# hukaixuan19970627/yolov5_obb

Hardware: AMD Instinct MI355X
Metric: val.py img/s (hot path: non_max_suppression_obb, bs16) + NMS ms/img @100k cand, DOTAv1.5 1024^2, 1/2/4/8 GPU (higher is better)
Workload: dtype f16; 1 GPU; DOTAv1.5 1024^2 bs16 (BASELINE metric; configs[1] thresholds): yolov5 OBB head output (16,64512,201) fp16, 4 distinct tensors rotated (cold: 1.66 GB working set) -> non_max_suppression_obb (conf .25, iou .45, multi_label, max_det 1500), val.py --task speed hot path = dt[2] of val.py; global_batch=16, anchors_per_image=64512, nc=16, detections_per_batch=3734, parallelism=dp1 (images sharded, no data-path collective)

## Files before the change

### include/obb_hip.h

```cpp
#ifndef OBB_HIP_H
#define OBB_HIP_H

#include <stddef.h>
#include <stdint.h>

#ifdef __cplusplus
extern "C" {
#endif

#define OBB_OK 0
#define OBB_ERR_BAD_ARG (-1)
#define OBB_ERR_WORKSPACE (-2)
#define OBB_ERR_LAUNCH (-3)
#define OBB_ERR_INTERNAL (-4)
#define OBB_ERR_NO_DEVICE (-5)

#define OBB_NMS_DROP_SMALL 1

const char* obb_version(void);
int obb_device_info(int* cu_count, int* wave_size, char* arch_name, int arch_name_len);
int obb_nms_set_max_grid(int max_workgroups);

#define OBB_PROF_STAGES 8
int obb_profile_enable(int on);
// ... 37 lines not shown
#define OBB_NMS_SORT_LDS_HINT 6144
#define OBB_NMS_SORT_LDS_MAX 8192
size_t obb_nms_obb_workspace_bytes(int64_t bs, int64_t cap_img, int64_t nc, int agnostic);
int obb_non_max_suppression_obb(const void* pred, int dtype, int64_t bs, int64_t A, int64_t no, float conf_thres,
                                float iou_thres, const int32_t* classes_host, int n_classes, int agnostic, int multi_label,
                                int64_t max_det, int64_t max_nms, float max_wh, const float* extra8, int64_t n_extra,
                                int64_t cap_img, int64_t expected_cand, float* out, int out_packed, int64_t* out_count,
                                int64_t* status, void* ws, size_t ws_bytes, void* stream);
int obb_non_max_suppression_obb_col(const void* pred, const void* objcol, int dtype, int64_t bs, int64_t A, int64_t no,
                                    float conf_thres, float iou_thres, const int32_t* classes_host, int n_classes, int agnostic,
                                    int multi_label, int64_t max_det, int64_t max_nms, float max_wh, const float* extra8,
                                    int64_t n_extra, int64_t cap_img, int64_t expected_cand, float* out, int out_packed,
                                    int64_t* out_count, int64_t* status, void* ws, size_t ws_bytes, void* stream);

size_t obb_nms_obb_state_bytes(int64_t bs);
int obb_non_max_suppression_obb_st(const void* pred, const void* objcol, int dtype, int64_t bs, int64_t A, int64_t no,
                                   float conf_thres, float iou_thres, const int32_t* classes_host, int n_classes, int agnostic,
                                   int multi_label, int64_t max_det, int64_t max_nms, float max_wh, const float* extra8,
                                   int64_t n_extra, int64_t cap_img, int64_t expected_cand, float* out, int out_packed,
                                   int64_t* out_count, int64_t* status, void* ws, size_t ws_bytes, void* state, size_t state_bytes,
                                   void* stream);

int obb_non_max_suppression_obb_head(int nl, const void* const* conv_out, int dtype, int64_t bs, int64_t na, int64_t no,
                                     const int64_t* ny, const int64_t* nx, const float* anchors_px_host, const float* strides_host,
                                     float conf_thres, float iou_thres, const int32_t* classes_host, int n_classes, int agnostic,
                                     int multi_label, int64_t max_det, int64_t max_nms, float max_wh, const float* extra8,
                                     int64_t n_extra, int64_t cap_img, int64_t expected_cand, float* out, int out_packed,
                                     int64_t* out_count, int64_t* status, void* ws, size_t ws_bytes, void* state, size_t state_bytes,
                                     void* stream);

// ... 84 lines not shown
```

### yolov5_obb_amd/_lib.py

```python
import ctypes as C
import os
import threading

import torch

_HERE = os.path.dirname(os.path.abspath(__file__))
LIB_PATH = os.environ.get("OBB_HIP_LIB") or os.path.join(_HERE, "libobb_hip.so")

OBB_OK = 0
OBB_NMS_DROP_SMALL = 1
_ERR = {-1: "bad argument", -2: "workspace missing or too small", -3: "kernel launch failed",
        -4: "internal error", -5: "no usable HIP device"}

_lib = None
_lock = threading.RLock()

_vp, _i64, _i32, _f32, _sz = C.c_void_p, C.c_int64, C.c_int, C.c_float, C.c_size_t

SIGNATURES = {
    "obb_version": (C.c_char_p, []),
    "obb_device_info": (_i32, [C.POINTER(_i32), C.POINTER(_i32), C.c_char_p, _i32]),
    "obb_nms_set_max_grid": (_i32, [_i32]),
    "obb_profile_enable": (_i32, [_i32]),
    "obb_profile_collect": (_i32, [_vp, _vp, _i32]),
# ... 3 lines not shown
    "obb_nms_poly_f32": (_i32, [_vp, _i64, _i64, _f32, _i64, _vp, _vp, _vp, _sz, _vp]),
    "obb_merge_nms_poly_f64": (_i32, [_vp, _i64, _vp, _vp, _i64, C.c_double, _vp, _vp, _vp, _sz, _vp]),
    "obb_merge_nms_poly_all_f64": (_i32, [_vp, _i64, _vp, _vp, _i64, C.c_double, _vp, _vp, _vp, _sz, _vp]),
    "obb_merge_nms_hbb_f64": (_i32, [_vp, _i64, _i64, _vp, _vp, _i64, C.c_double, _vp, _vp, _vp, _sz, _vp]),
    "obb_task1_parse_tiles": (_i64, [_vp, _i64, _i64, _vp, _vp, _vp, _vp, _vp, _vp]),
    "obb_task1_format_rows": (_i64, [_vp, _vp, _vp, _vp, _vp, _i64, _vp, _i64]),
    "obb_task1_parse_dets": (_i64, [_vp, _i64, _i64, _vp, _vp, _vp, _vp]),
    "obb_task1_parse_gt": (_i64, [_vp, _i64, _i64, _vp, _vp, _vp, _vp]),
    "obb_eval_best_gt_f64": (_i32, [_vp, _vp, _i64, _vp, _vp, _i64, _vp, _vp, _vp]),
    "obb_nms_obb_workspace_bytes": (_sz, [_i64, _i64, _i64, _i32]),
    "obb_non_max_suppression_obb": (_i32, [_vp, _i32, _i64, _i64, _i64, _f32, _f32, _vp, _i32, _i32, _i32, _i64, _i64, _f32,
                                           _vp, _i64, _i64, _i64, _vp, _i32, _vp, _vp, _vp, _sz, _vp]),
    "obb_non_max_suppression_obb_col": (_i32, [_vp, _vp, _i32, _i64, _i64, _i64, _f32, _f32, _vp, _i32, _i32, _i32, _i64, _i64, _f32,
                                               _vp, _i64, _i64, _i64, _vp, _i32, _vp, _vp, _vp, _sz, _vp]),
    "obb_nms_obb_state_bytes": (_sz, [_i64]),
    "obb_non_max_suppression_obb_st": (_i32, [_vp, _vp, _i32, _i64, _i64, _i64, _f32, _f32, _vp, _i32, _i32, _i32, _i64, _i64, _f32,
                                              _vp, _i64, _i64, _i64, _vp, _i32, _vp, _vp, _vp, _sz, _vp, _sz, _vp]),
    "obb_non_max_suppression_obb_head": (_i32, [_i32, _vp, _i32, _i64, _i64, _i64, _vp, _vp, _vp, _vp, _f32, _f32, _vp, _i32, _i32, _i32,
                                                _i64, _i64, _f32, _vp, _i64, _i64, _i64, _vp, _i32, _vp, _vp, _vp, _sz, _vp, _sz, _vp]),
    "obb_loss_workspace_bytes": (_sz, [_vp, _i64]),
    "obb_loss_build_targets": (_i32, [_vp, _vp, _i64, _i64, _vp, _vp, _sz, _vp]),
    "obb_loss_export_targets": (_i32, [_vp, _i64, _i32, _i64, _vp, _vp, _vp, _vp, _vp, _vp, _sz, _vp]),
    "obb_loss_forward": (_i32, [_vp, _vp, _i32, _vp, _i64, _i64, _vp, _vp, _sz, _vp]),
    "obb_loss_backward": (_i32, [_vp, _vp, _i32, _vp, _i64, _i64, _vp, _vp, _vp, _sz, _vp]),
    "obb_detect_decode": (_i32, [_vp, _i32, _i64, _i64, _i64, _i64, _i64, _vp, _f32, _vp, _vp, _i64, _i64, _vp]),
    "obb_detect_decode_col": (_i32, [_vp, _i32, _i64, _i64, _i64, _i64, _i64, _vp, _f32, _vp, _vp, _i64, _i64, _vp, _vp]),
    "obb_detect_decode_levels": (_i32, [_i32, _vp, _i32, _i64, _i64, _i64, _vp, _vp, _vp, _vp, _vp, _vp, _i64, _vp, _vp]),
    "obb_csl_encode_f32": (_i32, [_vp, _i64, _i32, C.c_double, C.c_double, _vp, _vp]),
    "obb_rbox2poly_f32": (_i32, [_vp, _i64, _i64, _vp, _vp, _vp]),
    "obb_val_postprocess_f32": (_i32, [_vp, _i64, _f32, _f32, _f32, _vp, _vp, _vp, _vp, _vp]),
# ... 202 lines not shown
```

### yolov5_obb_amd/csrc/nms.hip

```cpp
#include <hip/hip_runtime.h>
#include <cstring>
#include <stdint.h>
#include <stdlib.h>
#include <stdio.h>
#include <string.h>
#include <hip/hip_fp16.h>
#include "launch_once.h"
#include "obb_device.h"
#include "nms_core.h"
#include "nms_mk.h"
#include "obb_hip.h"
#include "psrs_sort.h"
#include "nms_small.h"
#include "segsort.h"

namespace obb {

enum { PROF_DECODE = 0, PROF_SEGSORT, PROF_PREP, PROF_STEPS, PROF_GATHER, PROF_NMS_SORT, PROF_NMS_PREP, PROF_NMS_STEPS, PROF_N };
struct ProfState {
  int on = 0;
  static constexpr int kMax = 8192;
  hipEvent_t ev0[kMax], ev1[kMax];
  int id[kMax];
  int created = 0, used = 0;
// ... 965 lines not shown
                                         out_packed, out_count, status, ws, ws_bytes, stream);
}

int obb_non_max_suppression_obb_col(const void* pred, const void* objcol, int dtype, int64_t bs, int64_t A, int64_t no,
                                    float conf_thres, float iou_thres, const int32_t* classes_host, int n_classes, int agnostic,
                                    int multi_label, int64_t max_det, int64_t max_nms, float max_wh, const float* extra8,
                                    int64_t n_extra, int64_t cap_img, int64_t expected_cand, float* out, int out_packed,
                                    int64_t* out_count, int64_t* status, void* ws, size_t ws_bytes, void* stream) {
  return run_nms_obb(pred, objcol, dtype, bs, A, no, conf_thres, iou_thres, classes_host, n_classes, agnostic, multi_label, max_det,
                     max_nms, max_wh, extra8, n_extra, cap_img, expected_cand, out, out_packed ? 1 : 0, out_count, status, ws, ws_bytes,
                     (hipStream_t)stream);
}

size_t obb_nms_obb_state_bytes(int64_t bs) { return bs < 1 ? 0 : obb_state_bytes(bs); }

int obb_non_max_suppression_obb_st(const void* pred, const void* objcol, int dtype, int64_t bs, int64_t A, int64_t no,
                                   float conf_thres, float iou_thres, const int32_t* classes_host, int n_classes, int agnostic,
                                   int multi_label, int64_t max_det, int64_t max_nms, float max_wh, const float* extra8,
                                   int64_t n_extra, int64_t cap_img, int64_t expected_cand, float* out, int out_packed,
                                   int64_t* out_count, int64_t* status, void* ws, size_t ws_bytes, void* state, size_t state_bytes,
                                   void* stream) {
  if (!state) return OBB_ERR_BAD_ARG;
  return run_nms_obb(pred, objcol, dtype, bs, A, no, conf_thres, iou_thres, classes_host, n_classes, agnostic, multi_label, max_det,
                     max_nms, max_wh, extra8, n_extra, cap_img, expected_cand, out, out_packed ? 1 : 0, out_count, status, ws, ws_bytes,
                     (hipStream_t)stream, state, state_bytes);
}

int obb_non_max_suppression_obb_head(int nl, const void* const* conv_out, int dtype, int64_t bs, int64_t na, int64_t no,
                                     const int64_t* ny, const int64_t* nx, const float* anchors_px_host, const float* strides_host,
                                     float conf_thres, float iou_thres, const int32_t* classes_host, int n_classes, int agnostic,
// ... 98 lines not shown
```

### yolov5_obb_amd/csrc/nms_small.h

```cpp
#pragma once

namespace obb {

#ifdef OBB_SMALL_TRACE
__device__ unsigned long long g_small_trace[2048 * 16];
__device__ unsigned long long g_small_trace_tail[2048 * 4];
__device__ unsigned long long g_small_trace2[2048 * 8];
#define STRACE(kind, ...) do { if (threadIdx.x == 0 && blockIdx.x < 2048) { const unsigned long long v_[] = {__VA_ARGS__}; unsigned long long* o_ = g_small_trace + blockIdx.x * 16; o_[0] = (kind); for (int z_ = 0; z_ < (int)(sizeof(v_) / 8) && z_ < 15; z_++) o_[1 + z_] = v_[z_]; } } while (0)
#endif
constexpr int kSmallMax = OBB_NMS_SMALL_SEG;
constexpr int kSmallWords = kSmallMax / 64;
constexpr int kSmallThreads = 512;
constexpr int kSmallWaves = kSmallThreads / 64;

struct SmallArgs {
  const float4* rec;
  const u64* alive;
  const int* seg_begin;
  const int* seg_end;
  int* keep_cnt;
  int64_t* keep_out;
  int* too_big;
  float thr;
  int max_keep;
// ... 52 lines not shown
    const bool apart = (d2 > rs * rs) & (fminf(a.w, cq.w) >= 2.34e-9f * d2);
    const bool row_ok = ((arow16 >> r) & 1u) != 0u && i0 + r < n;
    const bool pass = !apart & jv & (j > i0 + r) & row_ok;
    bits |= pass ? (1u << r) : 0u;
  }
  return bits;
}

template <class G>
struct SmallWave {
  float scr[G::SCR * 64];
  uint32_t q0[128], q1[128], q2[128];
};

template <class G, class FRONT>
__device__ __forceinline__ int small_segment(const SmallArgs& a, unsigned char* s_raw) {
  __shared__ int s_next, s_nkept, s_qcnt[kSmallWaves], s_qhead[kSmallWaves], s_qcnt2[kSmallWaves], s_last;
  __shared__ uint32_t s_kept[kSmallMax];
  __shared__ unsigned long long s_pk[kSmallMax];
  __shared__ uint32_t s_pv[kSmallMax];
  float4* s_rec = reinterpret_cast<float4*>(s_raw);
  u64* s_mask = reinterpret_cast<u64*>(s_rec + (size_t)kSmallMax * G::RECQ);
  u64* s_alive = s_mask + (size_t)kSmallMax * kSmallWords;
  SmallWave<G>* s_wave = reinterpret_cast<SmallWave<G>*>(s_alive + 8);
  const int tid = threadIdx.x, lane = tid & 63, wv = tid >> 6;
  int seg = (int)blockIdx.x - a.helpers, part = 0, np = 1, hbase = 0;
  if (seg < 0) {
    const int h = (int)blockIdx.x;
    if (h >= *a.help_cnt) {
#ifdef OBB_SMALL_TRACE
      STRACE(1ull, (unsigned long long)wall_clock64());
#endif
      return -1;
    }
    const int e = a.work[h];
    if (e < 0) return -1;
    seg = e & 0xffffff; part = e >> 24;
  }
  if (a.helpers > 0) { const int v = a.seg_np[seg]; if ((v & 255) > 1) { np = v & 255; hbase = v >> 8; } }
#ifdef OBB_SMALL_TRACE
  unsigned long long tt[8]; int ti_ = 0, nd0 = 0, nd1 = 0, nd2 = 0, nit = 0;
  unsigned long long acc_d0 = 0, acc_d1 = 0, acc_d2 = 0, acc_draw = 0, acc_l0 = 0, acc_l1 = 0, acc_l2 = 0;
#define SSTAMP() do { tt[ti_++] = wall_clock64(); } while (0)
// ... 267 lines not shown
    for (int k = tid; k < nk; k += kSmallThreads) a.keep_out[(size_t)sb + k] = (int64_t)(sb + (int)s_kept[k]);
    if (tid == 0) a.keep_cnt[seg] = nk;
  }
#ifdef OBB_SMALL_TRACE
  SSTAMP();
  STRACE(3ull, (unsigned long long)seg | ((unsigned long long)part << 24) | ((unsigned long long)np << 28), (unsigned long long)n, (unsigned long long)nk, tt[0], tt[1], tt[2], tt[3], tt[4], tt[5], tt[6], (unsigned long long)nit, (unsigned long long)nd0, (unsigned long long)nd1, (unsigned long long)nd2);
  if (tid == 0 && blockIdx.x < 2048) { unsigned long long* o_ = g_small_trace2 + blockIdx.x * 8; o_[0] = acc_d0; o_[1] = acc_d1; o_[2] = acc_d2; o_[3] = acc_draw; o_[4] = acc_l0; o_[5] = acc_l1; o_[6] = acc_l2; }
#endif
#undef SSTAMP
  return seg;
}

template <class G, class TAIL, class FRONT = SmallFromSort>
__global__ __launch_bounds__(kSmallThreads) void k_nms_small(SmallArgs a, typename TAIL::Args ta) {
  extern __shared__ __attribute__((aligned(16))) unsigned char s_raw[];
  const int seg = small_segment<G, FRONT>(a, s_raw);
  if (seg < 0) return;
  TAIL::run(a, ta, s_raw, seg);
}

static_assert((size_t)kSmallMax * RotGeom::RECQ * 16 + (size_t)kSmallMax * kSmallWords * 8 + 64 + sizeof(SmallWave<RotGeom>) * kSmallWaves +
              kSmallMax * 4 + kSmallMax * 12 + 256 <= 160 * 1024, "k_nms_small: LDS budget");
static_assert(kSmallMax % 64 == 0 && kSmallMax <= 65535, "k_nms_small: pair entries are (i << 16 | j)");

template <class G>
static size_t small_lds_bytes() {
  return (size_t)kSmallMax * G::RECQ * 16 + (size_t)kSmallMax * kSmallWords * 8 + 8 * 8 + sizeof(SmallWave<G>) * kSmallWaves;
}

}
```

### yolov5_obb_amd/csrc/nmsobb_impl.h

```cpp
#pragma once
#include "dtype_device.h"
#include "obb_device.h"
#include "segsort.h"

namespace obb {

struct ClassMask { unsigned long long w[4]; int all; };

template <typename T> __device__ __forceinline__ float mul_in_dtype(float a, float b);
template <> __device__ __forceinline__ float mul_in_dtype<float>(float a, float b) { return a * b; }
template <> __device__ __forceinline__ float mul_in_dtype<__half>(float a, float b) { return __half2float(__float2half_rn(a * b)); }
template <typename T> __device__ __forceinline__ float thr_in_dtype(float t);
template <> __device__ __forceinline__ float thr_in_dtype<float>(float t) { return t; }
template <> __device__ __forceinline__ float thr_in_dtype<__half>(float t) { return __half2float(__float2half_rn(t)); }

__device__ __forceinline__ unsigned long long argmax_key(float v, int i) {
  const uint32_t b = __float_as_uint(v + 0.0f);
  const uint32_t m = (v != v) ? 0xFFFFFFFFu : (b & 0x80000000u) ? ~b : (b | 0x80000000u);
  return ((unsigned long long)m << 32) | (unsigned long long)(0xFFFFFFFFu - (uint32_t)i);
}
template <int CTRL>
__device__ __forceinline__ unsigned long long dpp_max_u64(unsigned long long k) {
  const uint32_t lo = (uint32_t)__builtin_amdgcn_update_dpp(0, (int)(uint32_t)k, CTRL, 0xF, 0xF, true);
  const uint32_t hi = (uint32_t)__builtin_amdgcn_update_dpp(0, (int)(uint32_t)(k >> 32), CTRL, 0xF, 0xF, true);
// ... 96 lines not shown
#pragma unroll
  for (int k = 0; k < kDecCslRegs; k++) {
    const int bin = k * 16 + l16;
    r.csl[k] = (r.valid && bin < 180) ? ld_as_float<T>(csl + bin) : -__builtin_inff();
  }
#pragma unroll
  for (int g = 0; g < kDecClsRegs; g++) {
    const int c = g * 16 + l16;
    r.cls[g] = (r.valid && c < nc) ? ld_as_float<T>(base + 5 + c) : 0.f;
  }
#pragma unroll
  for (int k = 0; k < 4; k++) r.box[k] = r.valid ? ld_as_float<T>(base + k) : 0.f;
  return r;
}

template <typename T>
__global__ __launch_bounds__(kDecThreads) void k_decode(DecodeArgs a) {
  __shared__ float4 s_c0[kDecWaves][kDecStage], s_c1[kDecWaves][kDecStage];
  __shared__ unsigned long long s_key[kDecWaves][kDecStage];
  __shared__ int s_cnt[kDecWaves], s_base, s_n;
  __shared__ uint32_t s_row[kDecThreads * kDecMaxG];
  __shared__ float s_obj[kDecThreads * kDecMaxG];

  const T* pred = (const T*)a.pred;
  const int tid = threadIdx.x, lane = tid & 63, wv = tid >> 6;
  const int b = blockIdx.y;
  const int G = a.rows_per_thread;
  const float thr = thr_in_dtype<T>(a.conf_thres);
  const T* img = pred + (size_t)b * a.A * a.no;
  float4* cand = a.cand + (size_t)b * a.cap_img * 2;
  unsigned long long* keys = a.keys + (size_t)b * a.cap_img;
  uint32_t* vals = a.vals + (size_t)b * a.cap_img;
  float4* c0s = s_c0[wv]; float4* c1s = s_c1[wv]; unsigned long long* kys = s_key[wv];
  int staged = 0;
  int flags_seen = 0;
  if (tid == 0) s_n = 0;
  if (a.z_ticket != nullptr) {
    const long long i = ((long long)blockIdx.y * gridDim.x + blockIdx.x) * kDecThreads + tid, n = (long long)gridDim.x * gridDim.y * kDecThreads;
    if (i < a.n_ticket) a.z_ticket[i] = 0;
    for (long long k = i; k < a.n_bar16; k += n) a.z_bar16[k] = make_uint4(0u, 0u, 0u, 0u);
    for (long long k = i; k < a.n_alive16; k += n) a.z_alive16[k] = make_uint4(0u, 0u, 0u, 0u);
  }
  __syncthreads();

  auto write_out = [&](long long base, int count) {
    for (int i = lane; i < count; i += 64) {
      const long long slot = base + i;
      if (slot < a.cap_img) {
        cand[slot * 2] = c0s[i];
        cand[slot * 2 + 1] = c1s[i];
        keys[slot] = kys[i];
        vals[slot] = (uint32_t)slot;
      }
    }
  };
  auto flush_wave = [&]() {
    int base = 0;
    if (lane == 0) base = atomicAdd(&a.cnt[b * kCntPad], staged);
    base = __shfl(base, 0);
    write_out(base, staged);
    staged = 0;
  };

  float obj[kDecMaxG];
  auto row_of = [&](int q) -> long long { return ((long long)(q * (kDecThreads / 16) + (tid >> 4)) * gridDim.x + blockIdx.x) * 16 + (tid & 15); };
#pragma unroll
  for (int q = 0; q < kDecMaxG; q++) {
    const long long row = row_of(q);
    obj[q] = (q >= G || row >= a.A) ? 0.f
             : a.objcol ? ld_as_float<T>((const T*)a.objcol + (size_t)b * a.A + row)
                        : ld_as_float<T>(img + (size_t)row * a.no + 4);
  }
#pragma unroll
  for (int q = 0; q < kDecMaxG; q++) {
    const bool p = q < G && row_of(q) < a.A && obj[q] > thr;
    const unsigned long long mk = __ballot(p);
    if (mk) {
      int base = 0;
      if (lane == 0) base = atomicAdd(&s_n, __popcll(mk));
      base = __shfl(base, 0);
      if (p) {
        const int i = base + __popcll(mk & lanemask_lt());
        s_row[i] = (uint32_t)row_of(q);
        s_obj[i] = obj[q];
      }
    }
  }
  __syncthreads();
  const int n_rows = s_n;

  const int l16 = lane & 15, sub = lane >> 4;
  const int ncg = (a.nc + 15) >> 4;
  auto reduce_quad = [&](const DecQuad<T>& cur) {
    unsigned long long tk = argmax_key(cur.csl[0], l16);
#pragma unroll
    for (int k = 1; k < kDecCslRegs; k++) { const unsigned long long kk = argmax_key(cur.csl[k], k * 16 + l16); tk = kk > tk ? kk : tk; }
    float tv; int ti;
    argmax_unkey(row_max_u64(tk), tv, ti);
    const float theta = ((float)(ti - 90) / 180.0f) * 3.141592f;
    const float bx = cur.box[0], by = cur.box[1], bl = cur.box[2], bs_ = cur.box[3];
    const int bflags = cand_flags(bx, bl, bs_, a.win_lo, a.win_hi);
    const long long rw = (long long)cur.row;
    auto stage = [&](bool p, float conf, int c) {
      const unsigned long long pb = __ballot(p);
      const int np = __popcll(pb);
// ... 31 lines not shown
    for (int i = 0; i < kDecDepth; i++) {
      const int g = g0 + kDecWaves * i;
      if (g * 4 < n_rows) quads[i] = dec_load_quad<T>(img, a.no, a.nc, s_row, s_obj, g * 4 + sub, n_rows, l16);
    }
#pragma unroll
    for (int i = 0; i < kDecDepth; i++) {
      const int g = g0 + kDecWaves * i;
      if (g * 4 < n_rows) reduce_quad(quads[i]);
    }
  }

  {
    const int fl = (__ballot(flags_seen & kImgSmall) ? kImgSmall : 0) | (__ballot(flags_seen & kImgWide) ? kImgWide : 0);
    if (fl && lane == 0) atomicOr(&a.tiny[b], fl);
  }
  if (lane == 0) s_cnt[wv] = staged;
  __syncthreads();
  if (threadIdx.x == 0) {
    int tot = 0;
    for (int w = 0; w < kDecWaves; w++) tot += s_cnt[w];
    s_base = tot ? atomicAdd(&a.cnt[b * kCntPad], tot) : 0;
  }
  __syncthreads();
  int base = s_base;
  for (int w = 0; w < wv; w++) base += s_cnt[w];
  write_out(base, staged);
}

__global__ void k_append_extra(const float* __restrict__ extra8, int m, long long A, int nc, DecodeArgs a) {
  int i = blockIdx.x * blockDim.x + threadIdx.x;
  if (i >= m) return;
  const float* e = extra8 + (size_t)i * 8;
  const int b = (int)e[0];
  if (b < 0 || b >= a.bs) return;
  if (!(e[6] > a.conf_thres) || !class_allowed(a.cm, (int)e[7])) return;
  const int slot = atomicAdd(&a.cnt[b * kCntPad], 1);
  { const int fl = cand_flags(e[1], e[3], e[4], a.win_lo, a.win_hi); if (fl) atomicOr(&a.tiny[b], fl); }
  if (slot >= a.cap_img) return;
  const size_t g = (size_t)b * a.cap_img + slot;
  a.cand[g * 2] = make_float4(e[1], e[2], e[3], e[4]);
  a.cand[g * 2 + 1] = make_float4(e[5], e[6], e[7], 0.f);
// ... 682 lines not shown
    const long long max_det = ga.max_det;
    int cnt_c = 0;
    unsigned long long key = 0ull;
    uint32_t val = 0u;
    if (mine) {
      cnt_c = ldg_agent(a.keep_cnt + g * ncs + myc);
      size_t p = (size_t)sb_c + myk;
      if (p >= (size_t)a.n_pos) p = (size_t)a.n_pos - 1;
      val = ldg_agent(a.pub_val + p);
      key = ldg_agent(a.pub_key + p);
    }
    long long mx = 0;
    int tf = 0, big = 0;
    if (tid < 64) {
      for (int b2 = lane; b2 < ga.bs; b2 += 64) {
        const long long c = ga.cnt[b2 * kCntPad];
        if (c > mx) mx = c;
        const int t = ga.tiny[b2];
        tf |= t & kImgSmall;
        if ((t & kImgSmall) && !img_single_list(t)) tf |= 16;
      }
      if (tid == 0 && t2 == ga.bs - 1) big = ldg_agent(ga.info + 8);
    }
    if (max_det > 0 && cnt_c > max_det) cnt_c = (int)max_det;
    if (mine && myk == 0) { s_pre[myc + 1] = cnt_c; s_seg[myc] = sb_c; }
    if (tid == 0) s_pre[0] = 0;
    const int more = __syncthreads_or(cnt_c > spec ? 1 : 0);
    if (tid < 64) {
      int v[4], sum = 0, m = 0;
#pragma unroll
      for (int j = 0; j < 4; j++) { const int c = lane * 4 + j; v[j] = c < ncs ? s_pre[c + 1] : 0; sum += v[j]; m = v[j] > m ? v[j] : m; }
      int inc = sum;
#pragma unroll
// ... 118 lines not shown
#pragma unroll
    for (int d = 32; d >= 1; d >>= 1) { const long long o = __shfl_xor(mx, d); if (o > mx) mx = o; tf |= __shfl_xor(tf, d); }
    if (ga.clean_cnt != nullptr)
      for (int b2 = lane; b2 < ga.bs; b2 += 64) { ga.clean_cnt[b2 * kCntPad] = 0; ga.clean_tiny[b2] = 0; }
    if (lane == 0) {
      const int seg4 = ldg_agent(ga.info + 4);
      ga.status[0] = big ? -1 : (mx > ga.cap_img ? mx : 0);
      const long long small_seen = ((tf & kImgSmall) ? (1ll << 62) : 0ll) | ((tf & 16) ? (1ll << 61) : 0ll);
      ga.status[1] = mx | (((long long)(big > seg4 ? big : seg4) & 0x1fffffffll) << 32) | small_seen;
    }
  }
};
static_assert(SmallGather::kLdsBytes <= (size_t)kSmallMax * RotGeom::RECQ * 16 + (size_t)kSmallMax * kSmallWords * 8 + 64 + sizeof(SmallWave<RotGeom>) * kSmallWaves,
              "SmallGather: the merge lists live where the segment state was");

static inline size_t obb_state_bytes(int64_t bs) { return align_up((size_t)bs * kCntPad * 4 + (size_t)bs * 4); }

struct ObbCarve {
  float4* cand; unsigned long long *keys_a, *keys_b; uint32_t *vals_a, *vals_b; int* cnt; int *sort_begin, *sort_end;
  int *img_end, *mode, *tiny, *ticket;
  uint32_t* srs_hist;
  int* seg_size;
  int64_t* keep;
  Carve nms;
  void* nms_base;
  size_t total;
};

static inline int64_t round_cap(int64_t cap_img) { return (cap_img + 63) / 64 * 64; }

static int obb_carve(void* base, int64_t bs, int64_t cap_img, int64_t ncs, ObbCarve* cv) {
// ... 65 lines not shown
  {
    Carve& nv0 = cv.nms;
    const long long alive16 = lds_sort ? (long long)((((size_t)bs * cap_img) >> 6) + 8 + 1) / 2 : 0ll;
    if (kept) {
      d.z_ticket = cv.ticket; d.n_ticket = (int)(16 + bs + 1);
      d.z_bar16 = reinterpret_cast<uint4*>(nv0.bar); d.n_bar16 = (long long)(nv0.bar_bytes / 16);
      d.z_alive16 = reinterpret_cast<uint4*>(nv0.alive); d.n_alive16 = alive16;
    } else {
      k_reset_state<<<256, 256, 0, st>>>(cv.cnt, (int)(bs * kCntPad), cv.tiny, (int)bs, status, cv.ticket, (int)(16 + bs + 1),
                                         reinterpret_cast<uint4*>(nv0.bar), (long long)(nv0.bar_bytes / 16),
                                         reinterpret_cast<uint4*>(nv0.alive), alive16);
    }
  }
  d.rows_per_thread = (bs * A >= 4LL * kDecThreads * 480) ? 4 : (bs * A >= 2LL * kDecThreads * 480) ? 2 : 1;
  dim3 gd((unsigned)((A + kDecThreads * d.rows_per_thread - 1) / (kDecThreads * d.rows_per_thread)), (unsigned)bs);
  {
    ProfScope ps(PROF_DECODE, st);
    if (head) {
      rc = launch_decode_head(*head, d, dtype, st);
      if (rc) return rc;
    } else if (dtype == 0) k_decode<float><<<gd, kDecThreads, 0, st>>>(d);
    else k_decode<__half><<<gd, kDecThreads, 0, st>>>(d);
  }
  if (n_extra > 0 && extra8) k_append_extra<<<(unsigned)((n_extra + 255) / 256), 256, 0, st>>>(extra8, (int)n_extra, A, nc, d);
  if (small_hint && class_ok)
    k_tiny_cross<<<dim3(kTinyParts, (unsigned)bs), 256, 0, st>>>(cv.cand, cv.keys_a, cv.cnt, cap_img, max_wh, iou_thres, cv.tiny);
  const unsigned gs = (unsigned)((bs + 255) / 256);
  Carve& nv = cv.nms;
  const int64_t max_seg = (max_nms > 0 && max_nms < cap_img) ? max_nms : cap_img;
  const int nms_capmax = cap_max(bs * ncs);
  const int plan_chunk = kCapFirst < nms_capmax ? kCapFirst : nms_capmax;
  const bool small_nms = lds_sort && class_ok && seg_hint > 0 && seg_hint <= kSmallMax && iou_thres >= 0.f && bs * ncs <= 65535;
  const int plan_nb = (bs * ncs > 1 && !small_nms) ? nms_grid(bs * ncs, bs * max_seg, kCapFirst) : 0;
  const int helpers_env = [] { const char* e = getenv("OBB_NMS_SMALL_HELPERS"); const int v = (e && *e) ? atoi(e) : -1; return v > kSmallHelpMax ? kSmallHelpMax : v; }();
  const int self_env = [] { const char* e = getenv("OBB_NMS_SELF_SORT"); return (e && *e >= '0' && *e <= '2') ? *e - '0' : 2; }();
  const bool self_possible = small_nms && !out_packed && (int64_t)ncs * kSmallMax <= cap_img && self_env != 0;
  int helpers = 0;
  if (small_nms && !(self_possible && self_env == 2 && helpers_env < 0)) {
    const int64_t free_cus = (int64_t)hw_cu_count() - bs * ncs;
    helpers = helpers_env >= 0 ? helpers_env : (int)(free_cus < 0 ? 0 : (free_cus > kSmallHelpMax ? kSmallHelpMax : free_cus));
  }
// ... 2 lines not shown
  if (helpers > 0) {
    const size_t nseg_b = align_up((size_t)(bs * ncs) * 4), work_b = align_up((size_t)helpers * 4);
    const size_t main_b = align_up((size_t)bs * cap_img * kSmallWords * 8), help_b = align_up((size_t)helpers * kSmallMax * kSmallWords * 8);
    const size_t have = (size_t)((bs * ncs < (int64_t)cu_count()) ? bs * ncs : (int64_t)cu_count()) * (size_t)nv.ecap * 4;
    if (work_b + 2 * nseg_b + main_b + help_b > have) helpers = 0;
    else {
      char* p = reinterpret_cast<char*>(nv.edges);
      help_work = (int*)p; p += work_b;
      seg_np = (int*)p; p += nseg_b;
      seg_ticket = (int*)p; p += nseg_b;
      part_main = (u64*)p; p += main_b;
      part_help = (u64*)p;
    }
  }
  const bool self_sort = self_possible && helpers == 0;
  if (self_sort) {
  } else if (lds_sort) {
    ProfScope ps(PROF_SEGSORT, st);
    static OncePerDevice attr;
    const size_t lds = (size_t)kSortLdsMax * 12;
    if (const int attr_dev = attr.need(); attr_dev != OncePerDevice::kDone) {
      if (hipFuncSetAttribute((const void*)k_sort_prep_lds, hipFuncAttributeMaxDynamicSharedMemorySize, (int)lds) != hipSuccess)
        return OBB_ERR_LAUNCH;
      attr.mark(attr_dev);
    }
    const int parts = (class_ok && ncs >= 8) ? 4 : 1;
    k_sort_prep_lds<<<(unsigned)(bs * parts) + (plan_nb > 0 ? 1u : 0u), 1024, lds, st>>>(cv.cand, cv.keys_a, cv.vals_a, cv.keys_b, cv.vals_b, cv.cnt, cv.tiny, (int)bs, cap_img,
                                                   max_nms, class_ok, A, nc, ncs, agnostic ? 0.f : max_wh, cv.sort_begin, cv.sort_end,
                                                   cv.img_end, cv.mode, nv.seg_begin, nv.seg_end, nv.keep_cnt,
                                                   nv.rec, nv.alive, cv.ticket, plan_nb, plan_chunk, plan_nb > 0 ? nv.plan : nullptr,
// ... 47 lines not shown
  a.rows = nv.rows; a.nrows = nv.nrows; a.edges = nv.edges; a.nedges = nv.nedges;
  a.ecap = nv.ecap; a.n = (int)(bs * cap_img); a.capmax = cap_max(bs * ncs);
  a.max_keep = (int)max_det; a.window = nms_window(max_det); a.thr = iou_thres; a.cull = (iou_thres >= 0.f) ? 1 : 0;
  const bool fused_out = small_nms && !out_packed;
  if (small_nms) {
    ProfScope ps(PROF_STEPS, st);
    static OncePerDevice attr;
    const size_t lds = small_lds_bytes<RotGeom>();
    if (const int attr_dev = attr.need(); attr_dev != OncePerDevice::kDone) {
      if (hipFuncSetAttribute((const void*)k_nms_small<RotGeom, SmallNoTail>, hipFuncAttributeMaxDynamicSharedMemorySize, (int)lds) != hipSuccess ||
          hipFuncSetAttribute((const void*)k_nms_small<RotGeom, SmallGather>, hipFuncAttributeMaxDynamicSharedMemorySize, (int)lds) != hipSuccess ||
          hipFuncSetAttribute((const void*)k_nms_small<RotGeom, SmallGather, SmallSelfSort>, hipFuncAttributeMaxDynamicSharedMemorySize, (int)lds) != hipSuccess)
        return OBB_ERR_LAUNCH;
      attr.mark(attr_dev);
    }
    SmallArgs sa{};
    sa.rec = nv.rec; sa.alive = nv.alive; sa.seg_begin = nv.seg_begin; sa.seg_end = nv.seg_end; sa.keep_cnt = nv.keep_cnt;
    sa.keep_out = cv.keep; sa.too_big = cv.ticket + 8; sa.thr = iou_thres; sa.max_keep = (int)max_det;
    sa.ncs = ncs; sa.mode = cv.mode;
    sa.helpers = helpers; sa.help_cnt = cv.ticket + 12; sa.work = help_work; sa.seg_np = seg_np; sa.seg_ticket = seg_ticket;
    sa.part_main = part_main; sa.part_help = part_help;
    const unsigned gsmall = (unsigned)(bs * ncs + helpers);
    if (fused_out) {
      sa.keys_sorted = cv.keys_b; sa.vals_sorted = cv.vals_b; sa.pub_key = cv.keys_a; sa.pub_val = cv.vals_a; sa.n_pos = bs * cap_img;
      SmallGather::Args ga{};
      ga.cand = cv.cand; ga.cnt = cv.cnt; ga.tiny = cv.tiny; ga.info = cv.ticket; ga.ticket = cv.ticket + 16;
      ga.out = out; ga.out_count = out_count; ga.status = status; ga.cap_img = cap_img; ga.max_det = max_det; ga.bs = (int)bs;
      ga.clean_cnt = kept ? cv.cnt : nullptr; ga.clean_tiny = kept ? cv.tiny : nullptr;
      if (self_sort) {
        sa.pub_key = cv.keys_b; sa.pub_val = cv.vals_b; sa.keys_sorted = nullptr; sa.vals_sorted = nullptr;
        sa.keys_in = cv.keys_a; sa.cand = cv.cand; sa.cnt = cv.cnt; sa.tiny = cv.tiny; sa.cap_img = cap_img; sa.max_nms = max_nms; sa.A = A; sa.nc = nc;
        sa.class_offset = max_wh; sa.seg_max = cv.ticket + 4;
        k_nms_small<RotGeom, SmallGather, SmallSelfSort><<<gsmall, kSmallThreads, lds, st>>>(sa, ga);
      } else
      k_nms_small<RotGeom, SmallGather><<<gsmall, kSmallThreads, lds, st>>>(sa, ga);
    } else {
      k_nms_small<RotGeom, SmallNoTail><<<gsmall, kSmallThreads, lds, st>>>(sa, SmallNoTail::Args{});
    }
  } else {
    ProfScope ps(PROF_STEPS, st);
    rc = nms_steps(0, a, nv, bs * ncs, bs * max_seg, st, kNmsBarZeroed | ((lds_sort && plan_nb > 0) ? kNmsPlanned : 0));
    if (rc) return rc;
  }
  if (!fused_out) {
    ProfScope ps(PROF_GATHER, st);
    const unsigned gparts = expected_cand <= 2048 ? 1u : (unsigned)((expected_cand + 1023) / 1024 > 16 ? 16 : (expected_cand + 1023) / 1024);
    k_gather_out<<<dim3((unsigned)bs, gparts), 256, 0, st>>>(cv.cand, cv.vals_b, cv.keys_b, cv.keep, nv.seg_begin, nv.keep_cnt, cv.mode, ncs, max_det,
                                              out, out_count, cv.cnt, cap_img, status, nv.abort_flag, out_packed, cv.ticket, cv.tiny,
                                              kept ? cv.cnt : nullptr, kept ? cv.tiny : nullptr);
  }
// ... 5 lines not shown
```

Measured before the change: 143,300 img/s.

## Fuse decode filter and small-segment NMS into one persistent work-queue kernel

Adds a persistent kernel, launched with one workgroup per CU, that claims work items from an atomic counter. Items interleave per-image decode tiles with per-class NMS segments, and the next tile's objectness loads are prefetched. NMS segments spin on a per-image tiles-done counter, with a timeout fallback, so one image's NMS overlaps decode of later images, replacing separate decode and small-NMS launches. The last workgroup to leave resets the state counters, which replaces the zeroing the decode kernel did before. Risks are spin-wait stalls and lower occupancy from the larger combined LDS footprint.

After: 88050 img/s, median of 2. 38.6% lower.

```diff
diff --git a/include/obb_hip.h b/include/obb_hip.h
--- a/include/obb_hip.h
+++ b/include/obb_hip.h
@@ -75,6 +75,7 @@
                                     int64_t* out_count, int64_t* status, void* ws, size_t ws_bytes, void* stream);
 
 size_t obb_nms_obb_state_bytes(int64_t bs);
+int obb_debug_last_path(void);
 int obb_non_max_suppression_obb_st(const void* pred, const void* objcol, int dtype, int64_t bs, int64_t A, int64_t no,
                                    float conf_thres, float iou_thres, const int32_t* classes_host, int n_classes, int agnostic,
                                    int multi_label, int64_t max_det, int64_t max_nms, float max_wh, const float* extra8,
diff --git a/yolov5_obb_amd/_lib.py b/yolov5_obb_amd/_lib.py
--- a/yolov5_obb_amd/_lib.py
+++ b/yolov5_obb_amd/_lib.py
@@ -41,6 +41,7 @@
     "obb_non_max_suppression_obb_col": (_i32, [_vp, _vp, _i32, _i64, _i64, _i64, _f32, _f32, _vp, _i32, _i32, _i32, _i64, _i64, _f32,
                                                _vp, _i64, _i64, _i64, _vp, _i32, _vp, _vp, _vp, _sz, _vp]),
     "obb_nms_obb_state_bytes": (_sz, [_i64]),
+    "obb_debug_last_path": (_i32, []),
     "obb_non_max_suppression_obb_st": (_i32, [_vp, _vp, _i32, _i64, _i64, _i64, _f32, _f32, _vp, _i32, _i32, _i32, _i64, _i64, _f32,
                                               _vp, _i64, _i64, _i64, _vp, _i32, _vp, _vp, _vp, _sz, _vp, _sz, _vp]),
     "obb_non_max_suppression_obb_head": (_i32, [_i32, _vp, _i32, _i64, _i64, _i64, _vp, _vp, _vp, _vp, _f32, _f32, _vp, _i32, _i32, _i32,
diff --git a/yolov5_obb_amd/csrc/filter_nms.h b/yolov5_obb_amd/csrc/filter_nms.h
--- /dev/null
+++ b/yolov5_obb_amd/csrc/filter_nms.h
@@ -0,0 +1,128 @@
+#pragma once
+
+namespace obb {
+
+constexpr int kFusedG = 2;
+constexpr int kFusedLag = 1;
+constexpr long long kFusedSpinTicks = 20000000ll;
+
+struct FusedArgs {
+  int tiles, lead, bs, ncs, total;
+  int* work;
+  int* leave;
+  int* tiles_done;
+  int* info; int n_info;
+  int* cnt; int* tiny;
+};
+
+struct FusedState {
+  int* work; int* leave; int* tiles_done; int* info;
+  static size_t info_words(int64_t bs) { return (size_t)(16 + bs + 1); }
+  static size_t bytes(int64_t bs) { return 256 + 256 + align_up((size_t)bs * kCntPad * 4) + align_up(info_words(bs) * 4); }
+  static FusedState carve(void* base, int64_t bs) {
+    FusedState f;
+    char* p = (char*)base;
+    f.work = (int*)p; p += 256;
+    f.leave = (int*)p; p += 256;
+    f.tiles_done = (int*)p; p += align_up((size_t)bs * kCntPad * 4);
+    f.info = (int*)p;
+    return f;
+  }
+};
+
+__device__ __forceinline__ int fused_item(const FusedArgs& f, int i, int& g, int& sub) {
+  const int T = f.tiles, P = f.lead;
+  if (i < P * T) { g = i / T; sub = i - g * T; return 0; }
+  i -= P * T;
+  const int grp = f.ncs + T, nmix = f.bs - P;
+  if (i < nmix * grp) {
+    const int q = i / grp, r = i - q * grp;
+    if (r < f.ncs) { g = q; sub = r; return 1; }
+    g = q + P; sub = r - f.ncs; return 0;
+  }
+  i -= nmix * grp;
+  g = nmix + i / f.ncs; sub = i - (g - nmix) * f.ncs;
+  return 1;
+}
+
+template <typename T>
+__global__ __launch_bounds__(kSmallThreads) void k_filter_nms(DecodeArgs d, SmallArgs a, SmallGather::Args ga, FusedArgs f) {
+  extern __shared__ __attribute__((aligned(16))) unsigned char s_raw[];
+  __shared__ int s_item, s_ok;
+  DecLds& ds = *reinterpret_cast<DecLds*>(s_raw);
+  const int tid = threadIdx.x;
+  auto claim = [&]() { return __hip_atomic_fetch_add(f.work, 1, __ATOMIC_RELAXED, __HIP_MEMORY_SCOPE_AGENT); };
+  if (tid == 0) s_item = claim();
+  __syncthreads();
+  int cur = s_item;
+  float obj[kDecMaxG];
+  {
+    int g, sub;
+    if (cur < f.total && fused_item(f, cur, g, sub) == 0) dec_load_obj<T>(d, g, sub, f.tiles, obj);
+  }
+  while (cur < f.total) {
+    int g, sub;
+    const int kind = fused_item(f, cur, g, sub);
+    __syncthreads();
+    if (kind == 0) {
+      if (tid == 0) { s_item = claim(); ds.n = 0; }
+      __syncthreads();
+      const int nxt = s_item;
+      float objn[kDecMaxG];
+      int gn = 0, subn = 0;
+      const bool nxt_tile = nxt < f.total && fused_item(f, nxt, gn, subn) == 0;
+      if (nxt_tile) dec_load_obj<T>(d, gn, subn, f.tiles, objn);
+      dec_tile<T>(d, g, sub, f.tiles, obj, ds);
+      asm volatile("s_waitcnt vmcnt(0)" ::: "memory");
+      __syncthreads();
+      if (tid == 0) {
+        __builtin_amdgcn_fence(__ATOMIC_RELEASE, "agent");
+        asm volatile("s_waitcnt vmcnt(0)" ::: "memory");
+        __hip_atomic_fetch_add(f.tiles_done + g * kCntPad, 1, __ATOMIC_RELAXED, __HIP_MEMORY_SCOPE_AGENT);
+      }
+      if (nxt_tile) {
+#pragma unroll
+        for (int q = 0; q < kDecMaxG; q++) obj[q] = objn[q];
+      }
+      cur = nxt;
+      continue;
+    }
+    const int seg = g * f.ncs + sub;
+    if (tid == 0) {
+      int ok = 1;
+      if (__hip_atomic_load(f.tiles_done + g * kCntPad, __ATOMIC_RELAXED, __HIP_MEMORY_SCOPE_AGENT) < f.tiles) {
+        const unsigned long long t0 = wall_clock64();
+        while (__hip_atomic_load(f.tiles_done + g * kCntPad, __ATOMIC_RELAXED, __HIP_MEMORY_SCOPE_AGENT) < f.tiles) {
+          __builtin_amdgcn_s_sleep(2);
+          if ((long long)(wall_clock64() - t0) > kFusedSpinTicks) { ok = 0; break; }
+        }
+      }
+      __builtin_amdgcn_fence(__ATOMIC_ACQUIRE, "agent");
+      asm volatile("s_waitcnt vmcnt(0)" ::: "memory");
+      s_ok = ok;
+    }
+    __syncthreads();
+    if (s_ok) {
+      const int sg = small_segment<RotGeom, SmallSelfSort>(a, s_raw, a.helpers + seg);
+      if (sg >= 0) SmallGather::run(a, ga, s_raw, sg);
+    } else {
+      if (tid == 0) { stg_agent(a.keep_cnt + seg, 0); atomicMax(a.too_big, kSmallMax + 1); }
+      SmallGather::run(a, ga, s_raw, seg);
+    }
+    __syncthreads();
+    if (tid == 0) s_item = claim();
+    __syncthreads();
+    cur = s_item;
+    if (cur < f.total && fused_item(f, cur, g, sub) == 0) dec_load_obj<T>(d, g, sub, f.tiles, obj);
+  }
+  asm volatile("s_waitcnt vmcnt(0)" ::: "memory");
+  __syncthreads();
+  if (tid == 0) s_item = __hip_atomic_fetch_add(f.leave, 1, __ATOMIC_RELAXED, __HIP_MEMORY_SCOPE_AGENT);
+  __syncthreads();
+  if (s_item != (int)gridDim.x - 1) return;
+  if (tid == 0) { stg_agent(f.work, 0); stg_agent(f.leave, 0); }
+  for (int i = tid; i < f.bs; i += kSmallThreads) { stg_agent(f.tiles_done + i * kCntPad, 0); stg_agent(f.cnt + i * kCntPad, 0); stg_agent(f.tiny + i, 0); }
+  for (int i = tid; i < f.n_info; i += kSmallThreads) stg_agent(f.info + i, 0);
+}
+
+}
diff --git a/yolov5_obb_amd/csrc/nms.hip b/yolov5_obb_amd/csrc/nms.hip
--- a/yolov5_obb_amd/csrc/nms.hip
+++ b/yolov5_obb_amd/csrc/nms.hip
@@ -1003,6 +1003,8 @@
 
 size_t obb_nms_obb_state_bytes(int64_t bs) { return bs < 1 ? 0 : obb_state_bytes(bs); }
 
+int obb_debug_last_path(void) { return g_last_path; }
+
 int obb_non_max_suppression_obb_st(const void* pred, const void* objcol, int dtype, int64_t bs, int64_t A, int64_t no,
                                    float conf_thres, float iou_thres, const int32_t* classes_host, int n_classes, int agnostic,
                                    int multi_label, int64_t max_det, int64_t max_nms, float max_wh, const float* extra8,
diff --git a/yolov5_obb_amd/csrc/nms_small.h b/yolov5_obb_amd/csrc/nms_small.h
--- a/yolov5_obb_amd/csrc/nms_small.h
+++ b/yolov5_obb_amd/csrc/nms_small.h
@@ -90,7 +90,7 @@
 };
 
 template <class G, class FRONT>
-__device__ __forceinline__ int small_segment(const SmallArgs& a, unsigned char* s_raw) {
+__device__ __forceinline__ int small_segment(const SmallArgs& a, unsigned char* s_raw, int block) {
   __shared__ int s_next, s_nkept, s_qcnt[kSmallWaves], s_qhead[kSmallWaves], s_qcnt2[kSmallWaves], s_last;
   __shared__ uint32_t s_kept[kSmallMax];
   __shared__ unsigned long long s_pk[kSmallMax];
@@ -100,9 +100,9 @@
   u64* s_alive = s_mask + (size_t)kSmallMax * kSmallWords;
   SmallWave<G>* s_wave = reinterpret_cast<SmallWave<G>*>(s_alive + 8);
   const int tid = threadIdx.x, lane = tid & 63, wv = tid >> 6;
-  int seg = (int)blockIdx.x - a.helpers, part = 0, np = 1, hbase = 0;
+  int seg = block - a.helpers, part = 0, np = 1, hbase = 0;
   if (seg < 0) {
-    const int h = (int)blockIdx.x;
+    const int h = block;
     if (h >= *a.help_cnt) {
 #ifdef OBB_SMALL_TRACE
       STRACE(1ull, (unsigned long long)wall_clock64());
@@ -400,7 +400,7 @@
 template <class G, class TAIL, class FRONT = SmallFromSort>
 __global__ __launch_bounds__(kSmallThreads) void k_nms_small(SmallArgs a, typename TAIL::Args ta) {
   extern __shared__ __attribute__((aligned(16))) unsigned char s_raw[];
-  const int seg = small_segment<G, FRONT>(a, s_raw);
+  const int seg = small_segment<G, FRONT>(a, s_raw, (int)blockIdx.x);
   if (seg < 0) return;
   TAIL::run(a, ta, s_raw, seg);
 }
diff --git a/yolov5_obb_amd/csrc/nmsobb_impl.h b/yolov5_obb_amd/csrc/nmsobb_impl.h
--- a/yolov5_obb_amd/csrc/nmsobb_impl.h
+++ b/yolov5_obb_amd/csrc/nmsobb_impl.h
@@ -134,34 +134,45 @@
   return r;
 }
 
+struct DecLds {
+  float4 c0[kDecWaves][kDecStage], c1[kDecWaves][kDecStage];
+  unsigned long long key[kDecWaves][kDecStage];
+  int cnt[kDecWaves], base, n;
+  uint32_t row[kDecThreads * kDecMaxG];
+  float obj[kDecThreads * kDecMaxG];
+};
+
+__device__ __forceinline__ long long dec_row_of(int q, int tile, int ntiles) {
+  const int tid = threadIdx.x;
+  return ((long long)(q * (kDecThreads / 16) + (tid >> 4)) * ntiles + tile) * 16 + (tid & 15);
+}
 template <typename T>
-__global__ __launch_bounds__(kDecThreads) void k_decode(DecodeArgs a) {
-  __shared__ float4 s_c0[kDecWaves][kDecStage], s_c1[kDecWaves][kDecStage];
-  __shared__ unsigned long long s_key[kDecWaves][kDecStage];
-  __shared__ int s_cnt[kDecWaves], s_base, s_n;
-  __shared__ uint32_t s_row[kDecThreads * kDecMaxG];
-  __shared__ float s_obj[kDecThreads * kDecMaxG];
-
+__device__ __forceinline__ void dec_load_obj(const DecodeArgs& a, int b, int tile, int ntiles, float (&obj)[kDecMaxG]) {
+  const T* img = (const T*)a.pred + (size_t)b * a.A * a.no;
+  const int G = a.rows_per_thread;
+#pragma unroll
+  for (int q = 0; q < kDecMaxG; q++) {
+    const long long row = dec_row_of(q, tile, ntiles);
+    obj[q] = (q >= G || row >= a.A) ? 0.f
+             : a.objcol ? ld_as_float<T>((const T*)a.objcol + (size_t)b * a.A + row)
+                        : ld_as_float<T>(img + (size_t)row * a.no + 4);
+  }
+}
+
+template <typename T>
+__device__ __forceinline__ void dec_tile(const DecodeArgs& a, int b, int tile, int ntiles, const float (&obj)[kDecMaxG], DecLds& s) {
   const T* pred = (const T*)a.pred;
   const int tid = threadIdx.x, lane = tid & 63, wv = tid >> 6;
-  const int b = blockIdx.y;
   const int G = a.rows_per_thread;
   const float thr = thr_in_dtype<T>(a.conf_thres);
   const T* img = pred + (size_t)b * a.A * a.no;
   float4* cand = a.cand + (size_t)b * a.cap_img * 2;
   unsigned long long* keys = a.keys + (size_t)b * a.cap_img;
   uint32_t* vals = a.vals + (size_t)b * a.cap_img;
-  float4* c0s = s_c0[wv]; float4* c1s = s_c1[wv]; unsigned long long* kys = s_key[wv];
+  float4* c0s = s.c0[wv]; float4* c1s = s.c1[wv]; unsigned long long* kys = s.key[wv];
+  uint32_t* s_row = s.row; float* s_obj = s.obj;
   int staged = 0;
   int flags_seen = 0;
-  if (tid == 0) s_n = 0;
-  if (a.z_ticket != nullptr) {
-    const long long i = ((long long)blockIdx.y * gridDim.x + blockIdx.x) * kDecThreads + tid, n = (long long)gridDim.x * gridDim.y * kDecThreads;
-    if (i < a.n_ticket) a.z_ticket[i] = 0;
-    for (long long k = i; k < a.n_bar16; k += n) a.z_bar16[k] = make_uint4(0u, 0u, 0u, 0u);
-    for (long long k = i; k < a.n_alive16; k += n) a.z_alive16[k] = make_uint4(0u, 0u, 0u, 0u);
-  }
-  __syncthreads();
 
   auto write_out = [&](long long base, int count) {
     for (int i = lane; i < count; i += 64) {
@@ -182,33 +193,23 @@
     staged = 0;
   };
 
-  float obj[kDecMaxG];
-  auto row_of = [&](int q) -> long long { return ((long long)(q * (kDecThreads / 16) + (tid >> 4)) * gridDim.x + blockIdx.x) * 16 + (tid & 15); };
 #pragma unroll
   for (int q = 0; q < kDecMaxG; q++) {
-    const long long row = row_of(q);
-    obj[q] = (q >= G || row >= a.A) ? 0.f
-             : a.objcol ? ld_as_float<T>((const T*)a.objcol + (size_t)b * a.A + row)
-                        : ld_as_float<T>(img + (size_t)row * a.no + 4);
-  }
-#pragma unroll
-  for (int q = 0; q < kDecMaxG; q++) {
-    const bool p = q < G && row_of(q) < a.A && obj[q] > thr;
+    const bool p = q < G && dec_row_of(q, tile, ntiles) < a.A && obj[q] > thr;
     const unsigned long long mk = __ballot(p);
     if (mk) {
       int base = 0;
-      if (lane == 0) base = atomicAdd(&s_n, __popcll(mk));
+      if (lane == 0) base = atomicAdd(&s.n, __popcll(mk));
       base = __shfl(base, 0);
       if (p) {
         const int i = base + __popcll(mk & lanemask_lt());
-        s_row[i] = (uint32_t)row_of(q);
+        s_row[i] = (uint32_t)dec_row_of(q, tile, ntiles);
         s_obj[i] = obj[q];
       }
     }
   }
   __syncthreads();
-  const int n_rows = s_n;
-
+  const int n_rows = s.n;
   const int l16 = lane & 15, sub = lane >> 4;
   const int ncg = (a.nc + 15) >> 4;
   auto reduce_quad = [&](const DecQuad<T>& cur) {
@@ -270,17 +271,34 @@
     const int fl = (__ballot(flags_seen & kImgSmall) ? kImgSmall : 0) | (__ballot(flags_seen & kImgWide) ? kImgWide : 0);
     if (fl && lane == 0) atomicOr(&a.tiny[b], fl);
   }
-  if (lane == 0) s_cnt[wv] = staged;
+  if (lane == 0) s.cnt[wv] = staged;
   __syncthreads();
   if (threadIdx.x == 0) {
     int tot = 0;
-    for (int w = 0; w < kDecWaves; w++) tot += s_cnt[w];
-    s_base = tot ? atomicAdd(&a.cnt[b * kCntPad], tot) : 0;
+    for (int w = 0; w < kDecWaves; w++) tot += s.cnt[w];
+    s.base = tot ? atomicAdd(&a.cnt[b * kCntPad], tot) : 0;
   }
   __syncthreads();
-  int base = s_base;
-  for (int w = 0; w < wv; w++) base += s_cnt[w];
+  int base = s.base;
+  for (int w = 0; w < wv; w++) base += s.cnt[w];
   write_out(base, staged);
+}
+
+template <typename T>
+__global__ __launch_bounds__(kDecThreads) void k_decode(DecodeArgs a) {
+  __shared__ DecLds s;
+  const int tid = threadIdx.x;
+  if (tid == 0) s.n = 0;
+  if (a.z_ticket != nullptr) {
+    const long long i = ((long long)blockIdx.y * gridDim.x + blockIdx.x) * kDecThreads + tid, n = (long long)gridDim.x * gridDim.y * kDecThreads;
+    if (i < a.n_ticket) a.z_ticket[i] = 0;
+    for (long long k = i; k < a.n_bar16; k += n) a.z_bar16[k] = make_uint4(0u, 0u, 0u, 0u);
+    for (long long k = i; k < a.n_alive16; k += n) a.z_alive16[k] = make_uint4(0u, 0u, 0u, 0u);
+  }
+  __syncthreads();
+  float obj[kDecMaxG];
+  dec_load_obj<T>(a, (int)blockIdx.y, (int)blockIdx.x, (int)gridDim.x, obj);
+  dec_tile<T>(a, (int)blockIdx.y, (int)blockIdx.x, (int)gridDim.x, obj, s);
 }
 
 __global__ void k_append_extra(const float* __restrict__ extra8, int m, long long A, int nc, DecodeArgs a) {
@@ -993,9 +1011,9 @@
     int tf = 0, big = 0;
     if (tid < 64) {
       for (int b2 = lane; b2 < ga.bs; b2 += 64) {
-        const long long c = ga.cnt[b2 * kCntPad];
+        const long long c = ldg_agent(ga.cnt + b2 * kCntPad);
         if (c > mx) mx = c;
-        const int t = ga.tiny[b2];
+        const int t = ldg_agent(ga.tiny + b2);
         tf |= t & kImgSmall;
         if ((t & kImgSmall) && !img_single_list(t)) tf |= 16;
       }
@@ -1144,7 +1162,13 @@
 static_assert(SmallGather::kLdsBytes <= (size_t)kSmallMax * RotGeom::RECQ * 16 + (size_t)kSmallMax * kSmallWords * 8 + 64 + sizeof(SmallWave<RotGeom>) * kSmallWaves,
               "SmallGather: the merge lists live where the segment state was");
 
-static inline size_t obb_state_bytes(int64_t bs) { return align_up((size_t)bs * kCntPad * 4 + (size_t)bs * 4); }
+}
+#include "filter_nms.h"
+namespace obb {
+
+static inline size_t obb_state_head_bytes(int64_t bs) { return align_up((size_t)bs * kCntPad * 4 + (size_t)bs * 4); }
+static inline size_t obb_state_bytes(int64_t bs) { return obb_state_head_bytes(bs) + FusedState::bytes(bs); }
+static thread_local int g_last_path = 0;
 
 struct ObbCarve {
   float4* cand; unsigned long long *keys_a, *keys_b; uint32_t *vals_a, *vals_b; int* cnt; int *sort_begin, *sort_end;
@@ -1240,17 +1264,6 @@
   }
   d.rows_per_thread = (bs * A >= 4LL * kDecThreads * 480) ? 4 : (bs * A >= 2LL * kDecThreads * 480) ? 2 : 1;
   dim3 gd((unsigned)((A + kDecThreads * d.rows_per_thread - 1) / (kDecThreads * d.rows_per_thread)), (unsigned)bs);
-  {
-    ProfScope ps(PROF_DECODE, st);
-    if (head) {
-      rc = launch_decode_head(*head, d, dtype, st);
-      if (rc) return rc;
-    } else if (dtype == 0) k_decode<float><<<gd, kDecThreads, 0, st>>>(d);
-    else k_decode<__half><<<gd, kDecThreads, 0, st>>>(d);
-  }
-  if (n_extra > 0 && extra8) k_append_extra<<<(unsigned)((n_extra + 255) / 256), 256, 0, st>>>(extra8, (int)n_extra, A, nc, d);
-  if (small_hint && class_ok)
-    k_tiny_cross<<<dim3(kTinyParts, (unsigned)bs), 256, 0, st>>>(cv.cand, cv.keys_a, cv.cnt, cap_img, max_wh, iou_thres, cv.tiny);
   const unsigned gs = (unsigned)((bs + 255) / 256);
   Carve& nv = cv.nms;
   const int64_t max_seg = (max_nms > 0 && max_nms < cap_img) ? max_nms : cap_img;
@@ -1283,6 +1296,75 @@
     }
   }
   const bool self_sort = self_possible && helpers == 0;
+  g_last_path = 0;
+  const int fused_env = [] { const char* e = getenv("OBB_NMS_FUSED"); return (e && *e == '0') ? 0 : 1; }();
+  const bool fused = self_sort && kept && !head && n_extra == 0 && !(small_hint && class_ok) && fused_env && g_prof.on != 1;
+  auto small_args = [&](bool tail) {
+    SmallArgs sa{};
+    sa.rec = nv.rec; sa.alive = nv.alive; sa.seg_begin = nv.seg_begin; sa.seg_end = nv.seg_end; sa.keep_cnt = nv.keep_cnt;
+    sa.keep_out = cv.keep; sa.too_big = cv.ticket + 8; sa.thr = iou_thres; sa.max_keep = (int)max_det;
+    sa.ncs = ncs; sa.mode = cv.mode;
+    sa.helpers = helpers; sa.help_cnt = cv.ticket + 12; sa.work = help_work; sa.seg_np = seg_np; sa.seg_ticket = seg_ticket;
+    sa.part_main = part_main; sa.part_help = part_help;
+    if (!tail) return sa;
+    sa.keys_sorted = cv.keys_b; sa.vals_sorted = cv.vals_b; sa.pub_key = cv.keys_a; sa.pub_val = cv.vals_a; sa.n_pos = bs * cap_img;
+    if (self_sort) {
+      sa.pub_key = cv.keys_b; sa.pub_val = cv.vals_b; sa.keys_sorted = nullptr; sa.vals_sorted = nullptr;
+      sa.keys_in = cv.keys_a; sa.cand = cv.cand; sa.cnt = cv.cnt; sa.tiny = cv.tiny; sa.cap_img = cap_img; sa.max_nms = max_nms; sa.A = A; sa.nc = nc;
+      sa.class_offset = max_wh; sa.seg_max = cv.ticket + 4;
+    }
+    return sa;
+  };
+  auto gather_args = [&]() {
+    SmallGather::Args ga{};
+    ga.cand = cv.cand; ga.cnt = cv.cnt; ga.tiny = cv.tiny; ga.info = cv.ticket; ga.ticket = cv.ticket + 16;
+    ga.out = out; ga.out_count = out_count; ga.status = status; ga.cap_img = cap_img; ga.max_det = max_det; ga.bs = (int)bs;
+    ga.clean_cnt = kept ? cv.cnt : nullptr; ga.clean_tiny = kept ? cv.tiny : nullptr;
+    return ga;
+  };
+  if (fused) {
+    ProfScope ps(PROF_STEPS, st);
+    const size_t lds = small_lds_bytes<RotGeom>() > sizeof(DecLds) ? small_lds_bytes<RotGeom>() : sizeof(DecLds);
+    static OncePerDevice attr;
+    if (const int attr_dev = attr.need(); attr_dev != OncePerDevice::kDone) {
+      if (hipFuncSetAttribute((const void*)k_filter_nms<float>, hipFuncAttributeMaxDynamicSharedMemorySize, (int)lds) != hipSuccess ||
+          hipFuncSetAttribute((const void*)k_filter_nms<__half>, hipFuncAttributeMaxDynamicSharedMemorySize, (int)lds) != hipSuccess)
+        return OBB_ERR_LAUNCH;
+      attr.mark(attr_dev);
+    }
+    const FusedState fs = FusedState::carve((char*)state + obb_state_head_bytes(bs), bs);
+    cv.ticket = fs.info;
+    DecodeArgs df = d;
+    df.rows_per_thread = kFusedG;
+    df.z_ticket = nullptr; df.n_ticket = 0; df.z_bar16 = nullptr; df.n_bar16 = 0; df.z_alive16 = nullptr; df.n_alive16 = 0;
+    SmallArgs sa = small_args(true);
+    SmallGather::Args ga = gather_args();
+    ga.clean_cnt = nullptr; ga.clean_tiny = nullptr;
+    FusedArgs f;
+    f.tiles = (int)((A + kDecThreads * kFusedG - 1) / (kDecThreads * kFusedG));
+    f.lead = (int)(bs < kFusedLag + 1 ? bs : kFusedLag + 1);
+    f.bs = (int)bs; f.ncs = ncs;
+    if ((int64_t)f.tiles * bs + bs * ncs > 0x7fffffffLL - 4096) return OBB_ERR_BAD_ARG;
+    f.total = (int)(f.tiles * bs + bs * ncs);
+    f.work = fs.work; f.leave = fs.leave; f.tiles_done = fs.tiles_done; f.info = fs.info; f.n_info = (int)FusedState::info_words(bs);
+    f.cnt = cv.cnt; f.tiny = cv.tiny;
+    const unsigned grid = (unsigned)hw_cu_count();
+    if (dtype == 0) k_filter_nms<float><<<grid, kSmallThreads, lds, st>>>(df, sa, ga, f);
+    else k_filter_nms<__half><<<grid, kSmallThreads, lds, st>>>(df, sa, ga, f);
+    g_last_path = 1;
+    return hipGetLastError() == hipSuccess ? OBB_OK : OBB_ERR_LAUNCH;
+  }
+  {
+    ProfScope ps(PROF_DECODE, st);
+    if (head) {
+      rc = launch_decode_head(*head, d, dtype, st);
+      if (rc) return rc;
+    } else if (dtype == 0) k_decode<float><<<gd, kDecThreads, 0, st>>>(d);
+    else k_decode<__half><<<gd, kDecThreads, 0, st>>>(d);
+  }
+  if (n_extra > 0 && extra8) k_append_extra<<<(unsigned)((n_extra + 255) / 256), 256, 0, st>>>(extra8, (int)n_extra, A, nc, d);
+  if (small_hint && class_ok)
+    k_tiny_cross<<<dim3(kTinyParts, (unsigned)bs), 256, 0, st>>>(cv.cand, cv.keys_a, cv.cnt, cap_img, max_wh, iou_thres, cv.tiny);
   if (self_sort) {
   } else if (lds_sort) {
     ProfScope ps(PROF_SEGSORT, st);
@@ -1360,26 +1442,14 @@
         return OBB_ERR_LAUNCH;
       attr.mark(attr_dev);
     }
-    SmallArgs sa{};
-    sa.rec = nv.rec; sa.alive = nv.alive; sa.seg_begin = nv.seg_begin; sa.seg_end = nv.seg_end; sa.keep_cnt = nv.keep_cnt;
-    sa.keep_out = cv.keep; sa.too_big = cv.ticket + 8; sa.thr = iou_thres; sa.max_keep = (int)max_det;
-    sa.ncs = ncs; sa.mode = cv.mode;
-    sa.helpers = helpers; sa.help_cnt = cv.ticket + 12; sa.work = help_work; sa.seg_np = seg_np; sa.seg_ticket = seg_ticket;
-    sa.part_main = part_main; sa.part_help = part_help;
+    SmallArgs sa = small_args(fused_out);
     const unsigned gsmall = (unsigned)(bs * ncs + helpers);
     if (fused_out) {
-      sa.keys_sorted = cv.keys_b; sa.vals_sorted = cv.vals_b; sa.pub_key = cv.keys_a; sa.pub_val = cv.vals_a; sa.n_pos = bs * cap_img;
-      SmallGather::Args ga{};
-      ga.cand = cv.cand; ga.cnt = cv.cnt; ga.tiny = cv.tiny; ga.info = cv.ticket; ga.ticket = cv.ticket + 16;
-      ga.out = out; ga.out_count = out_count; ga.status = status; ga.cap_img = cap_img; ga.max_det = max_det; ga.bs = (int)bs;
-      ga.clean_cnt = kept ? cv.cnt : nullptr; ga.clean_tiny = kept ? cv.tiny : nullptr;
-      if (self_sort) {
-        sa.pub_key = cv.keys_b; sa.pub_val = cv.vals_b; sa.keys_sorted = nullptr; sa.vals_sorted = nullptr;
-        sa.keys_in = cv.keys_a; sa.cand = cv.cand; sa.cnt = cv.cnt; sa.tiny = cv.tiny; sa.cap_img = cap_img; sa.max_nms = max_nms; sa.A = A; sa.nc = nc;
-        sa.class_offset = max_wh; sa.seg_max = cv.ticket + 4;
+      SmallGather::Args ga = gather_args();
+      if (self_sort)
         k_nms_small<RotGeom, SmallGather, SmallSelfSort><<<gsmall, kSmallThreads, lds, st>>>(sa, ga);
-      } else
-      k_nms_small<RotGeom, SmallGather><<<gsmall, kSmallThreads, lds, st>>>(sa, ga);
+      else
+        k_nms_small<RotGeom, SmallGather><<<gsmall, kSmallThreads, lds, st>>>(sa, ga);
     } else {
       k_nms_small<RotGeom, SmallNoTail><<<gsmall, kSmallThreads, lds, st>>>(sa, SmallNoTail::Args{});
     }
```
